# epruesse/SINA

Hardware: AMD Instinct MI355X
Metric: aligned sequences/sec (whole node), 100k full-length 16S vs SILVA-NR-scale ref (higher is better)
Workload: dtype f32

## Files before the change

### sina_amd/csrc/api.hip

```cpp
#include <algorithm>
#include <cmath>
#include <cstdlib>
#include <cstring>

#include "common.h"
#include "ctx.h"

namespace sina_hip {

static thread_local std::string g_last_error;
static thread_local bool g_last_error_is_limit = false;
void set_error(const std::string &msg) {
    g_last_error = msg;
    g_last_error_is_limit = false;
}
void set_limit_error(const std::string &msg) {
    g_last_error = msg;
    g_last_error_is_limit = true;
}

int make_streams(sina_hip_ctx *c) {
    SH_CHECK(hipStreamCreateWithFlags(&c->stream, hipStreamNonBlocking));
    SH_CHECK(hipStreamCreateWithFlags(&c->stream_dp, hipStreamNonBlocking));
    return 0;
// ... 123 lines not shown

    const uint64_t tb_budget_cells = tb_plane_budget(c) / tb_cell_bytes(forbid);
    const uint32_t slots = dp_wave_slots(c, pl.geom.B);
    const uint32_t range_q = (uint32_t)strtoul(test_knob("dp_range_q").c_str(), nullptr, 10);
    auto nodes_of = [&](uint32_t q) { return g->node_off[q + 1] - g->node_off[q]; };
    HostPrep hp;
    for (uint32_t q0 = qa, q1; q0 < qb; q0 = q1) {
        q1 = dbg ? q0 + 1 : dp_cut_range(nodes_of, q0, qb, Lp, tb_budget_cells, slots);
        if (range_q != 0) q1 = std::min(q1, q0 + range_q);
        if (prep_range(g, qoff, q0, q1, Lp, pl.W, &hp, pp.on ? pp.kappa64 : 0.f, spill_q)) return 1;
        const uint32_t bq = q1 - q0;
        const uint64_t nbase = g->node_off[q0], nn = g->node_off[q1] - nbase;
        const uint64_t ebase = g->edge_off[q0], ne = g->edge_off[q1] - ebase;
        const uint64_t qbase = qoff[q0], nqm = qoff[q1] - qbase;
        if (c->qd.reserve(sizeof(QDesc) * bq) || c->rec.reserve(sizeof(uint4) * nn) || c->node_pos.reserve(4 * nn) ||
            c->pred.reserve(4 * std::max<uint64_t>(ne, 1)) || c->succ_minpos.reserve(4 * nn) ||
            c->qmask.reserve(nqm) || (pp.on && c->rgain.reserve(8 * nn)))
            return 1;
        hipStream_t s = c->stream;
        SH_CHECK(hipMemcpyAsync(c->qd.p, hp.qd.data(), sizeof(QDesc) * bq, hipMemcpyHostToDevice, s));
        SH_CHECK(hipMemcpyAsync(c->rec.p, hp.rec.data(), sizeof(uint4) * nn, hipMemcpyHostToDevice, s));
        SH_CHECK(hipMemcpyAsync(c->node_pos.p, g->node_pos + nbase, 4 * nn, hipMemcpyHostToDevice, s));
        if (ne) SH_CHECK(hipMemcpyAsync(c->pred.p, hp.pred.data(), 4 * ne, hipMemcpyHostToDevice, s));
        if (g->succ_minpos)
            SH_CHECK(hipMemcpyAsync(c->succ_minpos.p, g->succ_minpos + nbase, 4 * nn, hipMemcpyHostToDevice, s));
        SH_CHECK(hipMemcpyAsync(c->qmask.p, qmask + qbase, nqm, hipMemcpyHostToDevice, s));
        PrunePlan pp_launch = pp;
        if (!hp.rgain_ok) pp_launch.on = 0;
        if (pp.on) SH_CHECK(hipMemcpyAsync(c->rgain.p, hp.rgain.data(), 8 * nn, hipMemcpyHostToDevice, s));
        if (profile_batch) {
            if (!g->self_score16) SH_FAIL("align_graphs: node_score16 without self_score16");
            if (weighted_scheme(p)) SH_FAIL("align_graphs: a profile batch takes no positional weights (scoring_scheme_profile)");
            if (c->prof16.reserve(64 * std::max<uint64_t>(nn, 1)) || c->self16.reserve(64)) return 1;
            SH_CHECK(hipMemcpyAsync(c->prof16.p, g->node_score16 + 16 * nbase, 64 * nn, hipMemcpyHostToDevice, s));
            SH_CHECK(hipMemcpyAsync(c->self16.p, g->self_score16, 64, hipMemcpyHostToDevice, s));
        }
        DpLaunch l;
        l.qd = hp.qd.data();
// ... 360 lines not shown
```

### sina_amd/csrc/common.h

```cpp
#pragma once

#include <hip/hip_runtime.h>
#include <stdint.h>

#include <algorithm>
#include <atomic>
#include <mutex>
#include <string>
#include <vector>

#include <cstdio>
#include <cstdlib>
#include <ctime>

#include "sina_hip.h"

namespace sina_hip {

void set_error(const std::string &msg);
void set_limit_error(const std::string &msg);

inline std::string test_knob(const char *key) {
    const char *e = getenv("SINA_HIP_TEST");
    if (!e) return std::string();
// ... 115 lines not shown

struct QDesc {
    uint64_t node_off;
    uint64_t edge_off;
    uint64_t q_off;
    uint64_t tb_off;
    uint64_t spill_off;
    uint32_t N, L;
    uint32_t n_spill;
    uint32_t erec_off;
    uint32_t first_sink;
    uint32_t gmin;
};
static_assert(sizeof(QDesc) == 64, "uploaded as an array");

constexpr uint32_t kRecSink = 1u << 16;
constexpr uint32_t kRecFence = 1u << 17;
constexpr int kRecDistShift = 18;
constexpr uint32_t kRecDistFar = 63u;
constexpr uint32_t kRowNone = 0xFFFFFFFFu;
constexpr uint32_t kRowSpilled = 0x80000000u;
constexpr uint32_t kPredSpilled = 0x80000000u;
constexpr uint32_t kMaxSpillRows = 32768;
constexpr int kFarLds = 192;
__host__ __device__ inline uint32_t dp_slot_segment(uint32_t n_rows) {
    const uint32_t s = (n_rows + 15u) / 16u;
    return s < 256u ? 256u : s;
}

struct EdgeRec {
// ... 72 lines not shown
    const uint2 *reach;
    int prune;
    float prune_rho;
    uint32_t prune_amax;
    float scout_bias;
    float *scout_u;
    const uint16_t *chain_rows;
    const uint32_t *chain_sizes;
    uint32_t chain_ncap;
};

struct BtArgs {
    const QDesc *qd;
    const uint4 *rec;
    const uint32_t *pred;
    const uint32_t *node_pos;
    const void *tb;
    const DpResult *res;
    const float *weights;
    uint32_t n_weights;
    const uint32_t *wset;
    sina_hip_align_out *out;
    uint32_t *out_pos;
    uint32_t nq, width, Lp;
    float ms;
    int overhang;
    int lazy_sidx;
    const uint8_t *qmask;
    int lowercase;
    uint32_t asm_cap;
// ... 55 lines not shown
```

### sina_amd/csrc/ctx.h

```cpp
#pragma once

#include <atomic>
#include <algorithm>
#include <condition_variable>
#include <cmath>
#include <cstring>

#include "dp_plan.h"
#include "identity_plan.h"

struct sina_hip_store {
    sina_hip::DevBuf ref_ab, ref_off, idx_off, idx_ids;
    std::vector<uint64_t> ref_off_host;
    std::atomic<bool> ref_off_host_ready{false};
    uint32_t n_refs = 0, width = 0, k = 0, nofast = 0;
    uint64_t n_postings = 0, total_bases = 0;
    bool have_refs = false, have_index = false;
    sina_hip::DevBuf dense_id, dense_bits;
    uint32_t n_dense = 0, dense_words = 0;
    std::atomic<bool> dense_ready{false};
    sina_hip::DevBuf name_rank, name_inv;
    bool have_name_order = false;
    sina_hip::DevBuf pair_ent;
    uint32_t n_pair_ent = 0;
// ... 90 lines not shown

struct sina_hip_ctx {
    int device = 0;
    int n_cu = 256;
    hipStream_t stream = nullptr;
    hipStream_t stream_dp = nullptr;
    std::mutex mu;
    hipEvent_t ev[14];

    sina_hip_store *st = nullptr;
    bool owns_store = false;

    sina_hip::DevBuf qd, order, rec, node_pos, pred, succ_minpos, qmask, spill, edge, res, weights, out, out_pos, dbg;
    sina_hip::DevBuf prof16, self16;
    sina_hip::DevBuf rgain;
    sina_hip::DevBuf wset;
    sina_hip::DevBuf wide_in, wide_planes;
    uint64_t path_queries[sina_hip::kNumSlowPaths] = {};
    sina_hip::KernelUse use[sina_hip::kNumKernelUse];
    sina_hip::DevBuf k_big_keys, k_big_tmp;
    sina_hip::DevBuf scout, scout_u;
    sina_hip::HostBuf h_res;
    void *last_tb = nullptr;
    bool last_scout = false;
    uint32_t last_bq = 0, last_prune_step = 0;
    uint32_t last_kernel = 0;
    sina_hip::DevBuf k_qoff, k_scores, k_out_ids, k_out_scores, k_out_n, k_tmp0, k_tmp1, k_tmp2;
    sina_hip::DevBuf g_fam_ids, g_fam_off, g_tmp0, g_tmp1, g_tmp2, g_tmp3, g_sizes, g_wtab;
    sina_hip::DevBuf s_qab, s_qoff, s_cand, s_coff, s_out;
    sina_hip::DevBuf m_out, m_n;
    sina_hip::DevBuf r_keys, r_ids, r_scores, r_n, r_flag, r_cnt;
    sina_hip::InplaceCount inplace[sina_hip::kNumInplace] = {{24, sina_hip::kUsePairsInplace, 12},
                                                             {sina_hip::identity_row_bytes(1), sina_hip::kUseIdentityInplace, 13}};
    sina_hip::HostBuf h_out, h_out_pos;
    sina_hip::HostBuf h_stage[12];
    float wtab_fs_weight = NAN;
    uint32_t prof_ncap = 0;

    size_t lds_budget = 0;

    static constexpr int kNumScratch = 50;
    static_assert(kNumScratch <= 64, "sina_hip_store::cap_hint is too short");
    void scratch(sina_hip::DevBuf **all) {
        sina_hip::DevBuf *list[kNumScratch] = {&qd, &rec, &node_pos, &pred, &succ_minpos, &qmask, &spill, &res,
                                               &weights, &out, &out_pos, &k_qoff, &k_scores, &k_out_ids,
                                               &k_out_scores, &k_out_n, &k_tmp0, &k_tmp1, &k_tmp2, &g_fam_ids,
                                               &g_fam_off, &g_tmp0, &g_tmp1, &g_tmp2, &g_tmp3, &g_sizes, &g_wtab, &order,
                                               &s_qab, &s_qoff, &s_cand, &s_coff, &s_out, &edge, &prof16, &self16, &rgain,
                                               &scout, &scout_u, &wset, &m_out, &m_n, &r_keys, &r_ids, &r_scores, &r_n, &r_flag,
                                               &r_cnt, &inplace[sina_hip::kInplacePairs].rows, &inplace[sina_hip::kInplaceIdentity].rows};
        for (int i = 0; i < kNumScratch; i++) all[i] = list[i];
    }
    void publish_hints() {
        sina_hip::DevBuf *all[kNumScratch];
        scratch(all);
        for (int i = 0; i < kNumScratch; i++) {
            size_t seen = st->cap_hint[i].load(std::memory_order_relaxed);
            while (all[i]->cap > seen && !st->cap_hint[i].compare_exchange_weak(seen, all[i]->cap, std::memory_order_relaxed)) {
            }
        }
    }
    void bind_hints() {
        sina_hip::DevBuf *all[kNumScratch];
        scratch(all);
        for (int i = 0; i < kNumScratch; i++) all[i]->hint = &st->cap_hint[i];
        for (int i = 0; i < sina_hip::kNumInplace; i++) inplace[i].hint = &st->inplace_rows_hint[i];
    }
    int prewarm(int kind) {
        sina_hip::DevBuf *search[] = {&k_qoff, &k_scores, &k_out_ids, &k_out_scores, &k_out_n, &k_tmp0, &k_tmp1, &k_tmp2, &qmask,
                                      &s_qab, &r_keys, &r_ids, &r_scores, &r_n, &r_flag, &r_cnt};
        sina_hip::DevBuf *align[] = {&qd, &order, &rec, &node_pos, &pred, &succ_minpos, &qmask, &spill, &edge, &res, &weights, &out,
                                     &out_pos, &g_fam_ids, &g_fam_off, &g_tmp0, &g_tmp1, &g_tmp2, &g_tmp3, &g_sizes, &g_wtab, &rgain, &scout, &scout_u,
                                     &prof16, &self16, &wset, &inplace[sina_hip::kInplacePairs].rows, &inplace[sina_hip::kInplaceIdentity].rows};
        sina_hip::DevBuf *compare[] = {&s_qab, &s_qoff, &s_cand, &s_coff, &s_out, &m_out, &m_n, &r_keys, &r_ids, &r_scores, &r_n, &r_flag, &r_cnt};
        sina_hip::DevBuf **list = kind == 0 ? search : (kind == 1 ? align : compare);
        const size_t n = kind == 0 ? sizeof search / sizeof *search : (kind == 1 ? sizeof align / sizeof *align : sizeof compare / sizeof *compare);
        for (size_t i = 0; i < n; i++) {
            const size_t want = list[i]->hint ? list[i]->hint->load(std::memory_order_relaxed) : 0;
            if (want > list[i]->cap && list[i]->reserve_exact(want)) return 1;
        }
        for (auto &ic : inplace)
            if (kind == 1 && ic.h_rows.reserve(ic.hint->load(std::memory_order_relaxed))) return 1;
        return 0;
    }
    void free_all() {
        if (st && st->wedged.load(std::memory_order_relaxed)) return;
// ... 379 lines not shown
```

### sina_amd/csrc/dp_launch.hip

```cpp
#include <algorithm>
#include <cmath>
#include <cstdlib>
#include <cstring>

#include "common.h"
#include "ctx.h"

namespace sina_hip {

bool pick_geom(uint32_t maxL, DpGeom *g) {
    int t = 0, b = 0;
    if (const std::string ov = test_knob("geom"); ov.empty() || sscanf(ov.c_str(), "%d,%d", &t, &b) != 2) t = b = 0;
    return dp_geom_for(maxL, t, b, g);
}

int plan_dp(sina_hip_ctx *c, uint32_t maxL, DpPlan *pl) {
    DpGeom g;
    if (!pick_geom(maxL, &g)) SH_FAIL_LIMIT("align: query longer than SINA_HIP_MAX_QUERY_LEN bases");
    dp_ring_plan(g, c->lds_budget, pl);
    if (pl->W < 1) SH_FAIL("align: LDS cannot hold one DP row");
    return 0;
}

PrunePlan prune_plan(const sina_hip_align_params *p, float wmax, float wmin, uint32_t maxL, bool profile_batch) {
// ... 78 lines not shown
    }
    a->ms = -p->match_score;
    a->mms = -p->mismatch_score;
    a->gp = p->gap_penalty;
    a->gpe = p->gap_ext_penalty;
    a->prof16 = l.profile_batch ? c->prof16.as<float>() : nullptr;
    c->last_bq = l.bq;
    c->last_prune_step = pp.on ? pp.amax : 0u;
    a->reach = pp.on ? c->rgain.as<uint2>() : nullptr;
    a->prune = pp.on;
    a->prune_amax = pp.amax;
    a->below_init = (!weighted && !forbid && dp_below_init(sums.max_n, a->gp, a->gpe)) ? 1 : 0;
    b->qd = a->qd;
    b->rec = a->rec;
    b->pred = a->pred;
    b->node_pos = a->node_pos;
    b->res = a->res;
    b->weights = a->weights;
    b->n_weights = a->n_weights;
    b->wset = a->wset;
    b->out = c->out.as<sina_hip_align_out>();
    b->out_pos = c->out_pos.as<uint32_t>();
    b->nq = l.bq;
    b->width = l.width;
    b->Lp = (uint32_t)pl.geom.Lp();
    b->ms = a->ms;
    b->overhang = p->overhang;
    b->lazy_sidx = forbid ? 0 : 1;
    b->qmask = a->qmask;
    b->lowercase = p->lowercase;
// ... 267 lines not shown
```

### sina_amd/csrc/dp_plan.h

```cpp
#pragma once

#include <cassert>
#include <cmath>
#include <cstring>
#include <string_view>
#include <unordered_map>

#include "common.h"

namespace sina_hip {

enum DpKernelKind : uint32_t {
    kDpKernelNone = SINA_DP_KERNEL_NONE,
    kDpKernelSimple = SINA_DP_KERNEL_SIMPLE,
    kDpKernelSimpleSkip = SINA_DP_KERNEL_SIMPLE_SKIP,
    kDpKernelGenericBelow = SINA_DP_KERNEL_GENERIC_BELOW,
    kDpKernelGeneric = SINA_DP_KERNEL_GENERIC,
    kDpKernelWeighted = SINA_DP_KERNEL_WEIGHTED,
    kDpKernelForbid = SINA_DP_KERNEL_FORBID,
    kDpKernelWeightedForbid = SINA_DP_KERNEL_WEIGHTED_FORBID,
};
inline DpKernelKind dp_kernel_kind(bool weighted, bool forbid, bool below_init, float gp, float gpe, bool generic_only,
                                   bool profile_batch, bool prune_on, uint32_t n_strips) {
    if (!weighted && !forbid && below_init && gp >= gpe && !generic_only && !profile_batch)
// ... 203 lines not shown
    std::nth_element(ratios.begin(), ratios.begin() + (std::ptrdiff_t)at, ratios.end());
    const float rho_guard_seen = ratios[at] - 0.015f;
    if (!(rho_seen > 0.f)) return;
    *rho = rho_seen < *rho ? rho_seen : 0.5f * (*rho + rho_seen);
    *rho = std::min(0.99f, std::max(0.05f, *rho));
    *rho_guard = rho_guard_seen < *rho_guard ? rho_guard_seen : 0.5f * (*rho_guard + rho_guard_seen);
    *rho_guard = std::min(0.99f, std::max(0.05f, *rho_guard));
}

struct HostPrep {
    std::vector<QDesc> qd;
    std::vector<uint4> rec;
    std::vector<uint2> rgain;
    bool rgain_ok = true;
    std::vector<uint32_t> pred;
    std::vector<uint32_t> last;
};

inline int prep_range(const sina_hip_graph_batch *g, const uint64_t *qoff, uint32_t q0, uint32_t q1, int Lp, int W,
                       HostPrep *hp, float kappa64, uint32_t *spill_q) {
    const uint64_t nbase = g->node_off[q0], ebase = g->edge_off[q0];
    const uint64_t nn = g->node_off[q1] - nbase;
    hp->qd.resize(q1 - q0);
    hp->rec.resize(nn);
    hp->rgain.assign(kappa64 > 0.f ? nn : 0, uint2{0u, 0u});
    hp->rgain_ok = true;
    hp->pred.resize(g->edge_off[q1] - ebase + 8);
    uint64_t tb_cells = 0, spill_rows = 0;
    uint32_t erec_cursor = 0;
    for (uint32_t q = q0; q < q1; q++) {
        QDesc &d = hp->qd[q - q0];
        const uint64_t no = g->node_off[q], eo = g->edge_off[q];
        const uint32_t N = (uint32_t)(g->node_off[q + 1] - no);
        d.node_off = no - nbase;
        d.erec_off = erec_cursor;
        erec_cursor += dp_edge_entries(N);
        d.edge_off = eo - ebase;
        d.q_off = qoff[q] - qoff[q0];
        d.tb_off = tb_cells;
// ... 46 lines not shown
                for (int x = 0; x < W; x++)
                    if (free_at[x] <= m) {
                        slot = x;
                        break;
                    }
            if (slot >= 0) {
                free_at[slot] = last[m];
                rec[m].w = (uint32_t)slot;
            } else {
                rec[m].w = kRowSpilled | nsp++;
            }
        }
        for (uint32_t m = 0; m < N; m++) {
            uint32_t first_far = 0;
            uint32_t dist = po[m + 1] > po[m] ? 0u : kRecDistFar;
            for (uint32_t e = po[m]; e < po[m + 1]; e++) {
                const uint32_t p = g->pred[eo + e];
                const uint32_t pw = rec[p].w == kRowNone ? 0u : rec[p].w;
                const bool sp = (pw & kRowSpilled) != 0;
                if (sp && first_far == 0) first_far = e - po[m] + 1;
                dist = std::max(dist, m - p);
                hp->pred[d.edge_off + e] = p | ((pw & 0x7FFFu) << 16) | (sp ? kPredSpilled : 0u);
            }
            rec[m].z |= (first_far << 24) | (std::min(dist, kRecDistFar) << kRecDistShift);
        }
        if (nsp > kMaxSpillRows) {
            if (spill_q) *spill_q = q;
            SH_FAIL_LIMIT("align_graphs: too many spill rows for one query");
        }
        if (kappa64 > 0.f) {
            uint2 *rg = hp->rgain.data() + d.node_off;
            const uint32_t *pos = g->node_pos + no;
            bool ok = true;
            for (uint32_t m = 0; m < N && ok; m++) {
                if (m > 0 && pos[m] < pos[m - 1]) ok = false;
                for (uint32_t e = po[m]; e < po[m + 1] && ok; e++)
                    if (pos[g->pred[eo + e]] >= pos[m]) ok = false;
            }
            if (!ok) hp->rgain_ok = false;
// ... 44 lines not shown
```

### sina_amd/csrc/graph_build.hip

```cpp
#include <algorithm>
#include <cstring>
#include <type_traits>

#include "common.h"
#include "ctx.h"

namespace sina_hip {
namespace {

#ifndef SINA_GRAPH_THREADS
#define SINA_GRAPH_THREADS 512
#endif
#ifndef SINA_GRAPH_MINWAVES
#define SINA_GRAPH_MINWAVES 8
#endif
constexpr int kGT = SINA_GRAPH_THREADS;
constexpr uint32_t kNoPrev = 0xFFFFu;
constexpr int kMaxFam = kFamilyMax;
#ifndef SINA_GRAPH_KTC
#define SINA_GRAPH_KTC 128
#endif
#ifndef SINA_GRAPH_TNW
#define SINA_GRAPH_TNW 512
#endif
// ... 13 lines not shown
#define GP_FLUSH
#endif

struct GraphArgs {
    const uint32_t *ref_ab;
    const uint64_t *ref_off;
    const uint32_t *fam_ids;
    const uint64_t *fam_off;
    const uint64_t *pred_off;
    const float *wtab;
    uint4 *rec;
    uint32_t *node_pos;
    uint32_t *succ_min;
    uint32_t *far_mark;
    uint32_t *pred;
    uint32_t *sizes;
    uint16_t *chain_rows;
    uint32_t width, ncap;
    uint32_t tile_bytes;
    uint32_t bitmap_off;
    uint32_t member_off;
    uint32_t member_cap;
    uint32_t fam_cap;
    int W;
    int want_smin;
    uint2 *reach;
    float kappa64;
};

struct Member {
// ... 546 lines not shown
            }
            rec[i].w = w;
            if (in_lds) codeL[i] = w;
        }
        if (tid == 0) {
            sz[kBuiltN] = N;
            sz[kBuiltEdges] = E;
            sz[kBuiltSpill] = tot;
            sz[kBuiltStatus] = (tot > kMaxSpillRows) ? kBuiltSpillCap : 0u;
            sz[kBuiltFirstSink] = s_tmp[kGT / 64 + 1];
            sz[kBuiltChainLen] = mb[0].len;
        }
    }
    __syncthreads();
    GP(10)
    for (uint32_t i = tid; i < N; i += kGT) {
        const uint4 r = rec[i];
        const uint32_t np = r.z & 0xFFu;
        uint32_t first_far = 0;
        uint32_t dist = np ? 0u : kRecDistFar;
        for (uint32_t x = 0; x < np; x++) {
            const uint32_t pa = pred[r.x + x];
            uint32_t pw = in_lds ? codeL[pa] : rec[pa].w;
            if (pw == kRowNone) pw = 0;
            const bool sp = (pw & kRowSpilled) != 0;
            if (sp && first_far == 0) first_far = x + 1;
            dist = max(dist, i - pa);
            pred[r.x + x] = pa | ((pw & 0x7FFFu) << 16) | (sp ? kPredSpilled : 0u);
        }
        rec[i].z = r.z | (first_far << 24) | (min(dist, kRecDistFar) << kRecDistShift);
    }
    GP(11)
    if (a.reach != nullptr) {
        uint2 *rg = a.reach + (size_t)q * a.ncap;
        uint32_t *cw = in_lds ? codeL : (a.want_smin ? last : smin);
        if (tid == 0) s_tmp[kGT / 64 + 2] = 0xFFFFFFFFu;
        __syncthreads();
        for (uint32_t i = tid; i < N; i += kGT) {
            const uint32_t pos = node_pos[i];
            if (i > 0 && node_pos[i - 1] == pos) continue;
            uint32_t mx = 0;
            for (uint32_t j = i; j < N && node_pos[j] == pos; j++) {
                mx = max(mx, prune_gain_units(__uint_as_float(rec[j].y), a.kappa64));
                cw[j] = 0;
            }
// ... 63 lines not shown
    }
    uint32_t ncap = std::min<uint32_t>(65535, 12288);
    for (int attempt = 0;; attempt++) {
        uint64_t pred_total = 0;
        for (uint32_t q = 0; q < bq; q++) {
            bg->pred_off[q] = pred_total;
            pred_total += elems[q] + 8;
        }
        const size_t glds_tables = graph_lds_bytes(c->st->width, max_f);
        const size_t glds = graph_lds_total(c->st->width, max_f);
        if (glds > 160 * 1024) SH_FAIL_LIMIT("align_families: family too wide for the device DAG build");
        if (c->g_fam_ids.reserve(4 * std::max<uint64_t>(foff[bq], 1)) || c->g_fam_off.reserve(8 * ((uint64_t)bq + 1)) ||
            c->g_tmp1.reserve(8 * (uint64_t)bq) ||
            c->rec.reserve(sizeof(uint4) * (uint64_t)bq * ncap) || c->node_pos.reserve(4 * (uint64_t)bq * ncap) ||
            c->succ_minpos.reserve(4 * (uint64_t)bq * ncap) || c->g_tmp3.reserve(4 * (uint64_t)bq * ncap) ||
            c->pred.reserve(4 * pred_total) || c->g_sizes.reserve(4 * kBuiltWords * (uint64_t)bq) ||
            c->scout.reserve(2 * (uint64_t)bq * ncap) ||
            (kappa64 > 0.f && c->rgain.reserve(8 * (uint64_t)bq * ncap)))
            return 1;
        if (upload(c, 1, c->g_fam_ids.p, fam_ids + fam_off[q0], 4 * foff[bq], s) ||
            upload(c, 2, c->g_fam_off.p, foff.data(), 8 * ((uint64_t)bq + 1), s) ||
            upload(c, 3, c->g_tmp1.p, bg->pred_off.data(), 8 * (uint64_t)bq, s))
            return 1;
        GraphArgs ga;
        ga.ref_ab = c->st->ref_ab.as<uint32_t>();
        ga.ref_off = c->st->ref_off.as<uint64_t>();
        ga.fam_ids = c->g_fam_ids.as<uint32_t>();
        ga.fam_off = c->g_fam_off.as<uint64_t>();
        ga.pred_off = c->g_tmp1.as<uint64_t>();
        ga.wtab = c->g_wtab.as<float>();
        ga.rec = c->rec.as<uint4>();
        ga.node_pos = c->node_pos.as<uint32_t>();
        ga.succ_min = c->succ_minpos.as<uint32_t>();
        ga.far_mark = c->g_tmp3.as<uint32_t>();
        ga.pred = c->pred.as<uint32_t>();
        ga.sizes = c->g_sizes.as<uint32_t>();
        ga.chain_rows = c->scout.as<uint16_t>();
        ga.width = c->st->width;
        ga.ncap = ncap;
        ga.bitmap_off = (uint32_t)graph_bitmap_off(max_f);
        ga.tile_bytes = ga.bitmap_off;
        ga.member_off = (uint32_t)glds_tables;
        ga.member_cap = (uint32_t)graph_member_cap(max_f);
        ga.fam_cap = max_f;
        ga.W = W;
        ga.want_smin = want_smin ? 1 : 0;
        ga.reach = kappa64 > 0.f ? c->rgain.as<uint2>() : nullptr;
        ga.kappa64 = kappa64;
        if (allow_full_lds(reinterpret_cast<const void *>(family_graph_kernel))) return 1;
        bg->sizes.resize(kBuiltWords * (size_t)bq);
// ... 1 lines not shown
            heavy_launch hl(c, s, kHeavyGraph);
            SH_CHECK(hipEventRecord(c->ev[6], hl.stream()));
            hipLaunchKernelGGL(family_graph_kernel, dim3(bq), dim3(kGT), glds, hl.stream(), ga);
            SH_CHECK(hipGetLastError());
            SH_CHECK(hipEventRecord(c->ev[7], hl.stream()));
            if (hl.done()) return 1;
        }
        if (download(c, 4, c->g_sizes.p, 4 * kBuiltWords * (uint64_t)bq, s)) return 1;
        SH_CHECK(wait_stream(c, s));
        memcpy(bg->sizes.data(), c->h_stage[4].p, 4 * kBuiltWords * (uint64_t)bq);
        float gms = 0;
        SH_CHECK(hipEventElapsedTime(&gms, c->ev[6], c->ev[7]));
        {
            uint64_t bytes = 0;
            for (uint32_t q = 0; q < bq; q++)
                bytes += 4 * elems[q] + (uint64_t)bg->sizes[kBuiltWords * q + kBuiltN] * (16 + 4 + (kappa64 > 0.f ? 8 : 0)) +
                         4 * (uint64_t)bg->sizes[kBuiltWords * q + kBuiltEdges];
            std::lock_guard<std::mutex> slk(c->st->stats_mu);
            c->st->stats.graph_ms += gms;
            c->st->stats.graph_bytes += bytes;
            c->st->stats.graph_launches++;
        }
        uint32_t need_n = 0;
        for (uint32_t q = 0; q < bq; q++) {
            const uint32_t status = bg->sizes[kBuiltWords * q + kBuiltStatus];
            if (status == kBuiltNodeCap) need_n = std::max(need_n, bg->sizes[kBuiltWords * q + kBuiltN]);
            if (status == kBuiltSpillCap) SH_FAIL_LIMIT("align_families: too many spill rows for one query");
        }
        if (!need_n) break;
        if (attempt >= 3 || need_n > 65535u) SH_FAIL_LIMIT("align_families: family DAG exceeds device limits");
        ncap = std::min<uint32_t>(65535, need_n + need_n / 8 + 16);
// ... 113 lines not shown
```

### sina_amd/csrc/profile_build.hip

```cpp
#include <algorithm>
#include <cstring>
#include <limits>

#include "common.h"
#include "ctx.h"

namespace sina_hip {
namespace {

constexpr int kPT = 512;
constexpr uint32_t kTileMax = 6144;
constexpr uint32_t kLdsSlack = 256;

struct Shares {
    float v[6];
};
__host__ __device__ inline Shares shares_of_mask(uint32_t mask) {
    Shares b;
    for (int i = 0; i < 6; i++) b.v[i] = 0.f;
    const int order = ((mask >> 0) & 1) + ((mask >> 1) & 1) + ((mask >> 2) & 1) + ((mask >> 3) & 1);
    if (order > 0) {
        const float val = 1.f / (float)order;
        for (int i = 0; i < 4; i++)
            if (mask & (1u << i)) b.v[i] = val;
// ... 7 lines not shown
            if (i == j) res += match * a.v[i] * b.v[j];
            else res += mismatch * a.v[i] * b.v[j];
        }
    return res + gap * a.v[4] + gap_ext * a.v[5];
}

struct ProfileArgs {
    const uint32_t *ref_ab;
    const uint64_t *ref_off;
    const uint32_t *fam_ids;
    const uint64_t *fam_off;
    uint4 *rec;
    uint32_t *node_pos;
    uint32_t *succ_min;
    uint32_t *pred;
    float *prof16;
    uint32_t *sizes;
    uint32_t width, ncap, pred_stride;
    uint32_t tile_nodes;
    uint32_t bitmap_off;
    uint32_t member_off;
    float match, mismatch, gap, gap_ext;
};

struct PMember {
    uint64_t beg;
    uint32_t len;
    uint32_t cur, curn;
    uint32_t pad_;
};
// ... 76 lines not shown
            sz[kBuiltEdges] = sz[kBuiltSpill] = 0;
            sz[kBuiltStatus] = kBuiltNodeCap;
            sz[kBuiltFirstSink] = sz[kBuiltGmin] = 0;
        }
        return;
    }
    auto rank = [&](uint32_t pos) -> uint32_t {
        return (uint32_t)wrank[pos >> 5] + __popc(bitmap[pos >> 5] & ((1u << (pos & 31)) - 1u));
    };

    {
        uint4 *rec = a.rec + (size_t)q * a.ncap;
        uint32_t *node_pos = a.node_pos + (size_t)q * a.ncap;
        uint32_t *smin = a.succ_min + (size_t)q * a.ncap;
        uint32_t *pred = a.pred + (size_t)q * a.pred_stride;
        for (uint32_t w = tid; w < nwords; w += kPT) {
            uint32_t bits = bitmap[w], n = wrank[w];
            while (bits) {
                const uint32_t pos = w * 32u + (uint32_t)(__ffs(bits) - 1);
                bits &= bits - 1u;
                node_pos[n] = pos;
                if (n > 0) smin[n - 1] = pos;
                n++;
            }
        }
        for (uint32_t n = tid; n < N; n += kPT) {
            uint4 r;
            r.x = n > 0 ? n - 1u : 0u;
            r.y = 0u;
            r.z = (n > 0 ? 1u : 0u) | (n + 1 == N ? kRecSink : 0u) | ((n > 0 ? 1u : kRecDistFar) << kRecDistShift);
            r.w = kRowNone;
            rec[n] = r;
            if (n + 1 < N) pred[n] = n;
        }
        if (tid == 0) {
            smin[N - 1] = 1000000u;
            sz[kBuiltN] = N;
            sz[kBuiltEdges] = N - 1u;
            sz[kBuiltSpill] = 0;
            sz[kBuiltStatus] = 0;
            sz[kBuiltFirstSink] = N - 1u;
            sz[kBuiltGmin] = 0;
        }
    }

    float *prof = a.prof16 + 16 * ((size_t)q * a.ncap);
    for (uint32_t n0 = 0; n0 < N; n0 += T) {
// ... 166 lines not shown
        c->g_sizes.reserve(4 * kBuiltWords * (uint64_t)n))
        return 1;
    if (upload(c, 1, c->g_fam_ids.p, fam_ids + fam_off[q0], 4 * foff[n], s) ||
        upload(c, 2, c->g_fam_off.p, foff.data(), 8 * ((uint64_t)n + 1), s))
        return 1;
    if (allow_full_lds(reinterpret_cast<const void *>(family_profile_kernel))) return 1;
    uint32_t ncap = c->prof_ncap ? c->prof_ncap : 4096u;
    uint32_t max_n = 1;
    const uint32_t forced_tile = (uint32_t)strtoul(test_knob("profile_tile").c_str(), nullptr, 10);
    for (int attempt = 0;; attempt++) {
        ProfileLds lds;
        if (!profile_lds(c->st->width, max_f, ncap, forced_tile, &lds)) SH_FAIL_LIMIT("align_profiles: family too wide for the device profile build");
        const uint32_t pred_stride = ncap + 8;
        if (c->rec.reserve(sizeof(uint4) * (uint64_t)n * ncap) || c->node_pos.reserve(4 * (uint64_t)n * ncap) ||
            c->succ_minpos.reserve(4 * (uint64_t)n * ncap) || c->pred.reserve(4 * (uint64_t)n * pred_stride) ||
            c->prof16.reserve(64 * (uint64_t)n * ncap))
            return 1;
        ProfileArgs pa;
        pa.ref_ab = c->st->ref_ab.as<uint32_t>();
        pa.ref_off = c->st->ref_off.as<uint64_t>();
        pa.fam_ids = c->g_fam_ids.as<uint32_t>();
        pa.fam_off = c->g_fam_off.as<uint64_t>();
        pa.rec = c->rec.as<uint4>();
        pa.node_pos = c->node_pos.as<uint32_t>();
        pa.succ_min = c->succ_minpos.as<uint32_t>();
        pa.pred = c->pred.as<uint32_t>();
        pa.prof16 = c->prof16.as<float>();
        pa.sizes = c->g_sizes.as<uint32_t>();
        pa.width = c->st->width;
        pa.ncap = ncap;
        pa.pred_stride = pred_stride;
        pa.tile_nodes = lds.tile_nodes;
        pa.bitmap_off = lds.bitmap_off;
        pa.member_off = lds.member_off;
        pa.match = -p->match_score;
        pa.mismatch = -p->mismatch_score;
        pa.gap = p->gap_penalty;
        pa.gap_ext = p->gap_ext_penalty;
        {
            heavy_launch hl(c, s, kHeavyGraph);
            SH_CHECK(hipEventRecord(c->ev[6], hl.stream()));
// ... 9 lines not shown
        float gms = 0;
        SH_CHECK(hipEventElapsedTime(&gms, c->ev[6], c->ev[7]));
        uint32_t need_n = 0;
        uint64_t nodes = 0;
        max_n = 1;
        for (uint32_t q = 0; q < n; q++) {
            const uint32_t N = bg->sizes[kBuiltWords * q + kBuiltN];
            if (bg->sizes[kBuiltWords * q + kBuiltStatus] == kBuiltNodeCap) need_n = std::max(need_n, N);
            else nodes += N;
            max_n = std::max(max_n, N);
        }
        {
            std::lock_guard<std::mutex> slk(c->st->stats_mu);
            c->st->stats.graph_ms += gms;
            if (!need_n) {
                c->st->stats.graph_bytes += 4 * bases + nodes * (16 + 4 + 4 + 4 + 64);
                c->st->stats.graph_launches++;
            }
        }
        if (!need_n) break;
        if (attempt >= 3 || need_n > 65535u) SH_FAIL_LIMIT("align_profiles: family profile exceeds device limits (more than 65535 nodes)");
        ncap = std::min<uint32_t>(65535, need_n + need_n / 8 + 16);
    }
    c->prof_ncap = std::max(c->prof_ncap, std::min<uint32_t>(65535, max_n + max_n / 8 + 16));
    bg->ncap = ncap;
    bg->pred_off.resize(n);
    for (uint32_t q = 0; q < n; q++) bg->pred_off[q] = (uint64_t)q * (ncap + 8);
    return 0;
}

}
// ... 67 lines not shown
```

### sina_amd/csrc/traceback.hip

```cpp
#include <cstdlib>
#include <type_traits>

#include "common.h"
#include "dp_plan.h"

namespace sina_hip {

namespace {

template <bool LAZY>
struct BtDirect {
    using cell_t = typename std::conditional<LAZY, uint16_t, uint32_t>::type;
    static constexpr bool writes = true;
    const cell_t *tb;
    const uint4 *recs;
    const uint32_t *node_pos, *preds;
    uint32_t Lp;
    __device__ BtDirect(const BtArgs &a, const QDesc &d)
        : tb(reinterpret_cast<const cell_t *>(a.tb) + d.tb_off), recs(a.rec + d.node_off), node_pos(a.node_pos + d.node_off),
          preds(a.pred + d.edge_off), Lp(a.Lp) {}
    __device__ uint32_t cell(uint32_t row, uint32_t col) const { return (uint32_t)tb[(size_t)row * Lp + col]; }
    __device__ uint4 rec(uint32_t row) const {
        uint4 rx = recs[row];
        rx.w = node_pos[row];
        return rx;
    }
    __device__ uint32_t pred(uint32_t, uint32_t pb, uint32_t e) const { return preds[pb + e] & 0xffffu; }
};

constexpr int kBtRows = 64, kBtCols = 32;
template <bool LAZY>
struct BtWindow {
    using cell_t = typename BtDirect<LAZY>::cell_t;
    static constexpr uint32_t kAlign = 16 / sizeof(cell_t);
    struct Lds {
        cell_t cell[kBtRows][kBtCols];
        uint4 rec[kBtRows];
        uint4 pred[kBtRows];
    };
    BtDirect<LAZY> g;
    Lds &w;
    uint32_t N, lane;
    bool writes;
    uint32_t wr0 = 0x80000000u, wc0 = 0;
    __device__ BtWindow(const BtArgs &a, const QDesc &d, Lds &lds, uint32_t lane_)
        : g(a, d), w(lds), N(d.N), lane(lane_), writes(lane_ == 0) {}
    __device__ void refill(uint32_t row, uint32_t col) {
        __syncthreads();
        wr0 = row + 1 >= (uint32_t)kBtRows ? row + 1 - kBtRows : 0u;
        const uint32_t ctop = (col & ~(kAlign - 1)) + kAlign;
        wc0 = ctop >= (uint32_t)kBtCols ? ctop - kBtCols : 0u;
        const uint32_t x = wr0 + lane;
        if (x < N) {
            const uint4 *src = reinterpret_cast<const uint4 *>(g.tb + (size_t)x * g.Lp + wc0);
            uint4 *dst = reinterpret_cast<uint4 *>(&w.cell[lane][0]);
#pragma unroll
            for (uint32_t i = 0; i < kBtCols / kAlign; i++) dst[i] = src[i];
            const uint4 rx = g.rec(x);
            w.rec[lane] = rx;
            const uint32_t np = rx.z & 0xffu;
            uint4 pe = {0u, 0u, 0u, 0u};
            if (np > 0) pe.x = g.preds[rx.x];
            if (np > 1) pe.y = g.preds[rx.x + 1];
            if (np > 2) pe.z = g.preds[rx.x + 2];
            if (np > 3) pe.w = g.preds[rx.x + 3];
            w.pred[lane] = pe;
        }
        __syncthreads();
    }
    __device__ bool in_rows(uint32_t row) const { return row - wr0 < (uint32_t)kBtRows; }
    __device__ uint32_t cell(uint32_t row, uint32_t col) {
        if (!(in_rows(row) && col - wc0 < (uint32_t)kBtCols)) refill(row, col);
        return (uint32_t)w.cell[row - wr0][col - wc0];
    }
    __device__ uint4 rec(uint32_t row) const {
        if (in_rows(row)) return w.rec[row - wr0];
        return g.rec(row);
    }
    __device__ uint32_t pred(uint32_t row, uint32_t pb, uint32_t e) const {
        if (e < 4 && in_rows(row)) {
            const uint4 pe = w.pred[row - wr0];
            return (e == 0 ? pe.x : (e == 1 ? pe.y : (e == 2 ? pe.z : pe.w))) & 0xffffu;
        }
        return g.pred(row, pb, e);
    }
};

template <bool LAZY, class Mem>
__device__ __forceinline__ void walk_query(const BtArgs &a, uint32_t q, const QDesc &d, Mem &mem) {
    const DpResult r = a.res[q];
    sina_hip_align_out o;
    o.status = r.status;
    o.end_m = r.end_m;
    o.end_s = r.end_s;
    o.raw = r.raw;
    o.sum_weight = 0.f;
    o.aligned_bases = 0;
    o.cutoff_head = o.cutoff_tail = 0;
    o.n_out = 0;
    o.assembled = o.nast_total = o.nast_longest = o.nast_last_run = 0;
// ... 1 lines not shown
        if (mem.writes) a.out[q] = o;
        return;
    }
    uint32_t *out = a.out_pos + d.q_off;
    const uint32_t width = a.width;
    uint32_t m = r.end_m, s = r.end_s;
    uint32_t n = 0;
    const uint32_t send = d.L - 1;
    auto emit = [&](uint32_t p) {
        if (mem.writes) out[n] = p;
        n++;
    };

    const int tail = (int)(send - s);
    o.cutoff_tail = tail;
    uint32_t c = mem.cell(m, s);
    uint4 rm = mem.rec(m);
    if (tail && a.overhang != SINA_OVERHANG_REMOVE) {
        int pos = (a.overhang == SINA_OVERHANG_ATTACH) ? (int)(width - 1 - rm.w - (uint32_t)tail) : 0;
        for (int i = 0; i < tail; i++) {
            const int p = pos++;
            emit((uint32_t)(p > 0 ? p : 0));
        }
    }
    const uint8_t *qmb = a.qmask + d.q_off;
    const float *wts = a.weights;
    if (wts != nullptr && a.wset != nullptr) wts += (size_t)a.wset[q] * a.n_weights;
    auto mscore_at = [&](const uint4 &rx, uint32_t si) -> float {
        if (a.self16 != nullptr) return a.self16[qmb[si] & 0xfu];
        const float wgt = __uint_as_float(rx.y);
        if (wts != nullptr) {
            const uint32_t nw1 = a.n_weights - 1;
            return a.ms * wts[rx.w < nw1 ? rx.w : nw1] * wgt;
        }
        return a.ms * wgt;
    };
    unsigned int pos = width - 1 - rm.w;
    float sum_weight = 0.f;
    int aligned = 0;
    emit(pos);
    aligned++;
    sum_weight = sum_weight + mscore_at(rm, s);

    constexpr uint32_t ext_bit = LAZY ? kTb16Ext : kTbExt;
    auto gapm_idx = [&](uint32_t x, uint32_t col) -> uint32_t {
        for (uint32_t guard = 0; guard < 65536u; ++guard) {
            const uint32_t cx = mem.cell(x, col);
            const uint4 rx = mem.rec(x);
            const uint32_t np = rx.z & 0xffu;
            if (np == 0) return 0u;
            const uint32_t lastp = mem.pred(x, rx.x, np - 1);
            if (LAZY ? !(cx & kTb16XLast) : (cx & kTbOpLast) != 0) return lastp;
            x = lastp;
        }
        return 0u;
    };
    auto midx_raw = [&](uint32_t cc, uint32_t row, uint32_t pb) -> uint32_t {
        if (!LAZY) return cc >> 16;
        const uint32_t t = cc & kTbTypeMask;
        if (t == kTbIns) return row;
        if (t == kTbNone) return 0u;
        return mem.pred(row, pb, cc >> kTb16OrdShift);
    };
    auto sidx_of = [&](uint32_t cc, uint32_t row, uint32_t col) -> uint32_t {
        if (!LAZY) return cc & kTbSMask;
        const uint32_t t = cc & kTbTypeMask;
        if (t == kTbNone) return 0u;
        if (t == kTbMatch) return col - 1;
        if (t == kTbDel) return col;
        uint32_t k = col - 1;
        while (k > 0 && (mem.cell(row, k) & kTbTypeMask) == kTbIns) --k;
        return k;
    };
    auto is_deletion_at = [&](uint32_t cc, uint32_t col) -> bool {
        return LAZY ? (cc & kTbTypeMask) == kTbDel : (cc & kTbSMask) == col;
    };
    uint32_t npred_m = rm.z & 0xffu;
    while (s != 0 && npred_m != 0) {
        const uint32_t snew = sidx_of(c, m, s);
        const uint32_t vm = midx_raw(c, m, rm.x);
        m = (c & ext_bit) ? gapm_idx(vm, s) : vm;
        c = mem.cell(m, snew);
        if (snew != 0 && is_deletion_at(c, snew)) {
            const uint32_t vm2 = midx_raw(c, m, mem.rec(m).x);
            m = (c & ext_bit) ? gapm_idx(vm2, snew) : vm2;
            c = mem.cell(m, snew);
        }
        rm = mem.rec(m);
        npred_m = rm.z & 0xffu;
        pos = width - 1 - rm.w;
        while (s != snew) {
            --s;
            emit(pos);
            aligned++;
            sum_weight = sum_weight + mscore_at(rm, s);
        }
    }
    if (s != 0) {
        o.cutoff_head = (int)s;
        if (a.overhang == SINA_OVERHANG_ATTACH) {
            while (s-- != 0) {
                ++pos;
                emit((width - 1 < pos) ? width - 1 : pos);
// ... 160 lines not shown
```

Before: 294,600.

## Pack first four predecessors per node and fetch row state together in traceback

Adds a per-node pred4 array holding the first four predecessor indices as packed 16-bit values. It is built in the graph, profile and host prep paths and uploaded alongside the other graph buffers. Traceback now loads the cell, record and packed predecessors in one step, so the serial chain of dependent pred[] gathers becomes independent loads, and the LDS window shrinks from uint4 to uint2 per row. In exchange it costs extra memory, an extra host-to-device copy per range, and more work when building graphs.

```diff
diff --git a/sina_amd/csrc/api.hip b/sina_amd/csrc/api.hip
--- a/sina_amd/csrc/api.hip
+++ b/sina_amd/csrc/api.hip
@@ -161,7 +161,7 @@
         const uint64_t ebase = g->edge_off[q0], ne = g->edge_off[q1] - ebase;
         const uint64_t qbase = qoff[q0], nqm = qoff[q1] - qbase;
         if (c->qd.reserve(sizeof(QDesc) * bq) || c->rec.reserve(sizeof(uint4) * nn) || c->node_pos.reserve(4 * nn) ||
-            c->pred.reserve(4 * std::max<uint64_t>(ne, 1)) || c->succ_minpos.reserve(4 * nn) ||
+            c->pred.reserve(4 * std::max<uint64_t>(ne, 1)) || c->pred4.reserve(sizeof(uint2) * nn) || c->succ_minpos.reserve(4 * nn) ||
             c->qmask.reserve(nqm) || (pp.on && c->rgain.reserve(8 * nn)))
             return 1;
         hipStream_t s = c->stream;
@@ -169,6 +169,7 @@
         SH_CHECK(hipMemcpyAsync(c->rec.p, hp.rec.data(), sizeof(uint4) * nn, hipMemcpyHostToDevice, s));
         SH_CHECK(hipMemcpyAsync(c->node_pos.p, g->node_pos + nbase, 4 * nn, hipMemcpyHostToDevice, s));
         if (ne) SH_CHECK(hipMemcpyAsync(c->pred.p, hp.pred.data(), 4 * ne, hipMemcpyHostToDevice, s));
+        SH_CHECK(hipMemcpyAsync(c->pred4.p, hp.pred4.data(), sizeof(uint2) * nn, hipMemcpyHostToDevice, s));
         if (g->succ_minpos)
             SH_CHECK(hipMemcpyAsync(c->succ_minpos.p, g->succ_minpos + nbase, 4 * nn, hipMemcpyHostToDevice, s));
         SH_CHECK(hipMemcpyAsync(c->qmask.p, qmask + qbase, nqm, hipMemcpyHostToDevice, s));
diff --git a/sina_amd/csrc/common.h b/sina_amd/csrc/common.h
--- a/sina_amd/csrc/common.h
+++ b/sina_amd/csrc/common.h
@@ -153,6 +153,9 @@
 };
 static_assert(sizeof(QDesc) == 64, "uploaded as an array");
 
+__host__ __device__ inline uint2 pred4_pack(uint32_t p0, uint32_t p1, uint32_t p2, uint32_t p3) {
+    return uint2{(p0 & 0xffffu) | (p1 << 16), (p2 & 0xffffu) | (p3 << 16)};
+}
 constexpr uint32_t kRecSink = 1u << 16;
 constexpr uint32_t kRecFence = 1u << 17;
 constexpr int kRecDistShift = 18;
@@ -255,6 +258,7 @@
     const QDesc *qd;
     const uint4 *rec;
     const uint32_t *pred;
+    const uint2 *pred4;
     const uint32_t *node_pos;
     const void *tb;
     const DpResult *res;
diff --git a/sina_amd/csrc/ctx.h b/sina_amd/csrc/ctx.h
--- a/sina_amd/csrc/ctx.h
+++ b/sina_amd/csrc/ctx.h
@@ -128,6 +128,7 @@
     sina_hip::DevBuf qd, order, rec, node_pos, pred, succ_minpos, qmask, spill, edge, res, weights, out, out_pos, dbg;
     sina_hip::DevBuf prof16, self16;
     sina_hip::DevBuf rgain;
+    sina_hip::DevBuf pred4;
     sina_hip::DevBuf wset;
     sina_hip::DevBuf wide_in, wide_planes;
     uint64_t path_queries[sina_hip::kNumSlowPaths] = {};
@@ -153,7 +154,7 @@
 
     size_t lds_budget = 0;
 
-    static constexpr int kNumScratch = 50;
+    static constexpr int kNumScratch = 51;
     static_assert(kNumScratch <= 64, "sina_hip_store::cap_hint is too short");
     void scratch(sina_hip::DevBuf **all) {
         sina_hip::DevBuf *list[kNumScratch] = {&qd, &rec, &node_pos, &pred, &succ_minpos, &qmask, &spill, &res,
@@ -162,7 +163,7 @@
                                                &g_fam_off, &g_tmp0, &g_tmp1, &g_tmp2, &g_tmp3, &g_sizes, &g_wtab, &order,
                                                &s_qab, &s_qoff, &s_cand, &s_coff, &s_out, &edge, &prof16, &self16, &rgain,
                                                &scout, &scout_u, &wset, &m_out, &m_n, &r_keys, &r_ids, &r_scores, &r_n, &r_flag,
-                                               &r_cnt, &inplace[sina_hip::kInplacePairs].rows, &inplace[sina_hip::kInplaceIdentity].rows};
+                                               &r_cnt, &inplace[sina_hip::kInplacePairs].rows, &inplace[sina_hip::kInplaceIdentity].rows, &pred4};
         for (int i = 0; i < kNumScratch; i++) all[i] = list[i];
     }
     void publish_hints() {
@@ -183,7 +184,7 @@
     int prewarm(int kind) {
         sina_hip::DevBuf *search[] = {&k_qoff, &k_scores, &k_out_ids, &k_out_scores, &k_out_n, &k_tmp0, &k_tmp1, &k_tmp2, &qmask,
                                       &s_qab, &r_keys, &r_ids, &r_scores, &r_n, &r_flag, &r_cnt};
-        sina_hip::DevBuf *align[] = {&qd, &order, &rec, &node_pos, &pred, &succ_minpos, &qmask, &spill, &edge, &res, &weights, &out,
+        sina_hip::DevBuf *align[] = {&qd, &order, &rec, &node_pos, &pred, &pred4, &succ_minpos, &qmask, &spill, &edge, &res, &weights, &out,
                                      &out_pos, &g_fam_ids, &g_fam_off, &g_tmp0, &g_tmp1, &g_tmp2, &g_tmp3, &g_sizes, &g_wtab, &rgain, &scout, &scout_u,
                                      &prof16, &self16, &wset, &inplace[sina_hip::kInplacePairs].rows, &inplace[sina_hip::kInplaceIdentity].rows};
         sina_hip::DevBuf *compare[] = {&s_qab, &s_qoff, &s_cand, &s_coff, &s_out, &m_out, &m_n, &r_keys, &r_ids, &r_scores, &r_n, &r_flag, &r_cnt};
diff --git a/sina_amd/csrc/dp_launch.hip b/sina_amd/csrc/dp_launch.hip
--- a/sina_amd/csrc/dp_launch.hip
+++ b/sina_amd/csrc/dp_launch.hip
@@ -116,6 +116,7 @@
     b->qd = a->qd;
     b->rec = a->rec;
     b->pred = a->pred;
+    b->pred4 = c->pred4.as<uint2>();
     b->node_pos = a->node_pos;
     b->res = a->res;
     b->weights = a->weights;
diff --git a/sina_amd/csrc/dp_plan.h b/sina_amd/csrc/dp_plan.h
--- a/sina_amd/csrc/dp_plan.h
+++ b/sina_amd/csrc/dp_plan.h
@@ -241,6 +241,7 @@
     std::vector<uint2> rgain;
     bool rgain_ok = true;
     std::vector<uint32_t> pred;
+    std::vector<uint2> pred4;
     std::vector<uint32_t> last;
 };
 
@@ -250,6 +251,7 @@
     const uint64_t nn = g->node_off[q1] - nbase;
     hp->qd.resize(q1 - q0);
     hp->rec.resize(nn);
+    hp->pred4.resize(nn);
     hp->rgain.assign(kappa64 > 0.f ? nn : 0, uint2{0u, 0u});
     hp->rgain_ok = true;
     hp->pred.resize(g->edge_off[q1] - ebase + 8);
@@ -326,8 +328,10 @@
         for (uint32_t m = 0; m < N; m++) {
             uint32_t first_far = 0;
             uint32_t dist = po[m + 1] > po[m] ? 0u : kRecDistFar;
+            uint32_t p4[4] = {0u, 0u, 0u, 0u};
             for (uint32_t e = po[m]; e < po[m + 1]; e++) {
                 const uint32_t p = g->pred[eo + e];
+                if (e - po[m] < 4u) p4[e - po[m]] = p;
                 const uint32_t pw = rec[p].w == kRowNone ? 0u : rec[p].w;
                 const bool sp = (pw & kRowSpilled) != 0;
                 if (sp && first_far == 0) first_far = e - po[m] + 1;
@@ -335,6 +339,7 @@
                 hp->pred[d.edge_off + e] = p | ((pw & 0x7FFFu) << 16) | (sp ? kPredSpilled : 0u);
             }
             rec[m].z |= (first_far << 24) | (std::min(dist, kRecDistFar) << kRecDistShift);
+            hp->pred4[d.node_off + m] = pred4_pack(p4[0], p4[1], p4[2], p4[3]);
         }
         if (nsp > kMaxSpillRows) {
             if (spill_q) *spill_q = q;
diff --git a/sina_amd/csrc/graph_build.hip b/sina_amd/csrc/graph_build.hip
--- a/sina_amd/csrc/graph_build.hip
+++ b/sina_amd/csrc/graph_build.hip
@@ -51,6 +51,7 @@
     uint32_t *succ_min;
     uint32_t *far_mark;
     uint32_t *pred;
+    uint2 *pred4;
     uint32_t *sizes;
     uint16_t *chain_rows;
     uint32_t width, ncap;
@@ -627,11 +628,13 @@
     }
     __syncthreads();
     GP(10)
+    uint2 *pred4 = a.pred4 + (size_t)q * a.ncap;
     for (uint32_t i = tid; i < N; i += kGT) {
         const uint4 r = rec[i];
         const uint32_t np = r.z & 0xFFu;
         uint32_t first_far = 0;
         uint32_t dist = np ? 0u : kRecDistFar;
+        uint32_t p4[4] = {0u, 0u, 0u, 0u};
         for (uint32_t x = 0; x < np; x++) {
             const uint32_t pa = pred[r.x + x];
             uint32_t pw = in_lds ? codeL[pa] : rec[pa].w;
@@ -640,8 +643,13 @@
             if (sp && first_far == 0) first_far = x + 1;
             dist = max(dist, i - pa);
             pred[r.x + x] = pa | ((pw & 0x7FFFu) << 16) | (sp ? kPredSpilled : 0u);
+            if (x == 0) p4[0] = pa;
+            else if (x == 1) p4[1] = pa;
+            else if (x == 2) p4[2] = pa;
+            else if (x == 3) p4[3] = pa;
         }
         rec[i].z = r.z | (first_far << 24) | (min(dist, kRecDistFar) << kRecDistShift);
+        pred4[i] = pred4_pack(p4[0], p4[1], p4[2], p4[3]);
     }
     GP(11)
     if (a.reach != nullptr) {
@@ -735,7 +743,7 @@
             c->g_tmp1.reserve(8 * (uint64_t)bq) ||
             c->rec.reserve(sizeof(uint4) * (uint64_t)bq * ncap) || c->node_pos.reserve(4 * (uint64_t)bq * ncap) ||
             c->succ_minpos.reserve(4 * (uint64_t)bq * ncap) || c->g_tmp3.reserve(4 * (uint64_t)bq * ncap) ||
-            c->pred.reserve(4 * pred_total) || c->g_sizes.reserve(4 * kBuiltWords * (uint64_t)bq) ||
+            c->pred.reserve(4 * pred_total) || c->pred4.reserve(sizeof(uint2) * (uint64_t)bq * ncap) || c->g_sizes.reserve(4 * kBuiltWords * (uint64_t)bq) ||
             c->scout.reserve(2 * (uint64_t)bq * ncap) ||
             (kappa64 > 0.f && c->rgain.reserve(8 * (uint64_t)bq * ncap)))
             return 1;
@@ -755,6 +763,7 @@
         ga.succ_min = c->succ_minpos.as<uint32_t>();
         ga.far_mark = c->g_tmp3.as<uint32_t>();
         ga.pred = c->pred.as<uint32_t>();
+        ga.pred4 = c->pred4.as<uint2>();
         ga.sizes = c->g_sizes.as<uint32_t>();
         ga.chain_rows = c->scout.as<uint16_t>();
         ga.width = c->st->width;
@@ -786,7 +795,7 @@
         {
             uint64_t bytes = 0;
             for (uint32_t q = 0; q < bq; q++)
-                bytes += 4 * elems[q] + (uint64_t)bg->sizes[kBuiltWords * q + kBuiltN] * (16 + 4 + (kappa64 > 0.f ? 8 : 0)) +
+                bytes += 4 * elems[q] + (uint64_t)bg->sizes[kBuiltWords * q + kBuiltN] * (16 + 4 + 8 + (kappa64 > 0.f ? 8 : 0)) +
                          4 * (uint64_t)bg->sizes[kBuiltWords * q + kBuiltEdges];
             std::lock_guard<std::mutex> slk(c->st->stats_mu);
             c->st->stats.graph_ms += gms;
diff --git a/sina_amd/csrc/profile_build.hip b/sina_amd/csrc/profile_build.hip
--- a/sina_amd/csrc/profile_build.hip
+++ b/sina_amd/csrc/profile_build.hip
@@ -45,6 +45,7 @@
     uint32_t *node_pos;
     uint32_t *succ_min;
     uint32_t *pred;
+    uint2 *pred4;
     float *prof16;
     uint32_t *sizes;
     uint32_t width, ncap, pred_stride;
@@ -151,6 +152,7 @@
         uint32_t *node_pos = a.node_pos + (size_t)q * a.ncap;
         uint32_t *smin = a.succ_min + (size_t)q * a.ncap;
         uint32_t *pred = a.pred + (size_t)q * a.pred_stride;
+        uint2 *pred4 = a.pred4 + (size_t)q * a.ncap;
         for (uint32_t w = tid; w < nwords; w += kPT) {
             uint32_t bits = bitmap[w], n = wrank[w];
             while (bits) {
@@ -168,6 +170,7 @@
             r.z = (n > 0 ? 1u : 0u) | (n + 1 == N ? kRecSink : 0u) | ((n > 0 ? 1u : kRecDistFar) << kRecDistShift);
             r.w = kRowNone;
             rec[n] = r;
+            pred4[n] = pred4_pack(n > 0 ? n - 1u : 0u, 0u, 0u, 0u);
             if (n + 1 < N) pred[n] = n;
         }
         if (tid == 0) {
@@ -364,6 +367,7 @@
         const uint32_t pred_stride = ncap + 8;
         if (c->rec.reserve(sizeof(uint4) * (uint64_t)n * ncap) || c->node_pos.reserve(4 * (uint64_t)n * ncap) ||
             c->succ_minpos.reserve(4 * (uint64_t)n * ncap) || c->pred.reserve(4 * (uint64_t)n * pred_stride) ||
+            c->pred4.reserve(sizeof(uint2) * (uint64_t)n * ncap) ||
             c->prof16.reserve(64 * (uint64_t)n * ncap))
             return 1;
         ProfileArgs pa;
@@ -375,6 +379,7 @@
         pa.node_pos = c->node_pos.as<uint32_t>();
         pa.succ_min = c->succ_minpos.as<uint32_t>();
         pa.pred = c->pred.as<uint32_t>();
+        pa.pred4 = c->pred4.as<uint2>();
         pa.prof16 = c->prof16.as<float>();
         pa.sizes = c->g_sizes.as<uint32_t>();
         pa.width = c->st->width;
@@ -414,7 +419,7 @@
             std::lock_guard<std::mutex> slk(c->st->stats_mu);
             c->st->stats.graph_ms += gms;
             if (!need_n) {
-                c->st->stats.graph_bytes += 4 * bases + nodes * (16 + 4 + 4 + 4 + 64);
+                c->st->stats.graph_bytes += 4 * bases + nodes * (16 + 4 + 4 + 4 + 8 + 64);
                 c->st->stats.graph_launches++;
             }
         }
diff --git a/sina_amd/csrc/traceback.hip b/sina_amd/csrc/traceback.hip
--- a/sina_amd/csrc/traceback.hip
+++ b/sina_amd/csrc/traceback.hip
@@ -7,6 +7,17 @@
 namespace sina_hip {
 
 namespace {
+
+struct BtAt {
+    uint32_t c;
+    uint4 r;
+    uint2 p4;
+    __device__ uint32_t npred() const { return r.z & 0xffu; }
+    __device__ uint32_t pred_near(uint32_t e) const {
+        const uint32_t w = (e & 2u) ? p4.y : p4.x;
+        return (e & 1u) ? w >> 16 : w & 0xffffu;
+    }
+};
 
 template <bool LAZY>
 struct BtDirect {
@@ -14,18 +25,28 @@
     static constexpr bool writes = true;
     const cell_t *tb;
     const uint4 *recs;
+    const uint2 *pred4;
     const uint32_t *node_pos, *preds;
     uint32_t Lp;
     __device__ BtDirect(const BtArgs &a, const QDesc &d)
-        : tb(reinterpret_cast<const cell_t *>(a.tb) + d.tb_off), recs(a.rec + d.node_off), node_pos(a.node_pos + d.node_off),
-          preds(a.pred + d.edge_off), Lp(a.Lp) {}
+        : tb(reinterpret_cast<const cell_t *>(a.tb) + d.tb_off), recs(a.rec + d.node_off), pred4(a.pred4 + d.node_off),
+          node_pos(a.node_pos + d.node_off), preds(a.pred + d.edge_off), Lp(a.Lp) {}
     __device__ uint32_t cell(uint32_t row, uint32_t col) const { return (uint32_t)tb[(size_t)row * Lp + col]; }
     __device__ uint4 rec(uint32_t row) const {
         uint4 rx = recs[row];
         rx.w = node_pos[row];
         return rx;
     }
-    __device__ uint32_t pred(uint32_t, uint32_t pb, uint32_t e) const { return preds[pb + e] & 0xffffu; }
+    __device__ BtAt at(uint32_t row, uint32_t col) const {
+        BtAt x;
+        x.c = cell(row, col);
+        x.r = recs[row];
+        x.r.w = node_pos[row];
+        x.p4 = pred4[row];
+        asm volatile("" : "+v"(x.c), "+v"(x.r.x), "+v"(x.r.y), "+v"(x.r.z), "+v"(x.r.w), "+v"(x.p4.x), "+v"(x.p4.y));
+        return x;
+    }
+    __device__ uint32_t pred_far(uint32_t pb, uint32_t e) const { return preds[pb + e] & 0xffffu; }
 };
 
 constexpr int kBtRows = 64, kBtCols = 32;
@@ -36,7 +57,7 @@
     struct Lds {
         cell_t cell[kBtRows][kBtCols];
         uint4 rec[kBtRows];
-        uint4 pred[kBtRows];
+        uint2 pred[kBtRows];
     };
     BtDirect<LAZY> g;
     Lds &w;
@@ -56,15 +77,8 @@
             uint4 *dst = reinterpret_cast<uint4 *>(&w.cell[lane][0]);
 #pragma unroll
             for (uint32_t i = 0; i < kBtCols / kAlign; i++) dst[i] = src[i];
-            const uint4 rx = g.rec(x);
-            w.rec[lane] = rx;
-            const uint32_t np = rx.z & 0xffu;
-            uint4 pe = {0u, 0u, 0u, 0u};
-            if (np > 0) pe.x = g.preds[rx.x];
-            if (np > 1) pe.y = g.preds[rx.x + 1];
-            if (np > 2) pe.z = g.preds[rx.x + 2];
-            if (np > 3) pe.w = g.preds[rx.x + 3];
-            w.pred[lane] = pe;
+            w.rec[lane] = g.rec(x);
+            w.pred[lane] = g.pred4[x];
         }
         __syncthreads();
     }
@@ -73,17 +87,14 @@
         if (!(in_rows(row) && col - wc0 < (uint32_t)kBtCols)) refill(row, col);
         return (uint32_t)w.cell[row - wr0][col - wc0];
     }
-    __device__ uint4 rec(uint32_t row) const {
-        if (in_rows(row)) return w.rec[row - wr0];
-        return g.rec(row);
-    }
-    __device__ uint32_t pred(uint32_t row, uint32_t pb, uint32_t e) const {
-        if (e < 4 && in_rows(row)) {
-            const uint4 pe = w.pred[row - wr0];
-            return (e == 0 ? pe.x : (e == 1 ? pe.y : (e == 2 ? pe.z : pe.w))) & 0xffffu;
-        }
-        return g.pred(row, pb, e);
-    }
+    __device__ BtAt at(uint32_t row, uint32_t col) {
+        BtAt x;
+        x.c = cell(row, col);
+        x.r = w.rec[row - wr0];
+        x.p4 = w.pred[row - wr0];
+        return x;
+    }
+    __device__ uint32_t pred_far(uint32_t pb, uint32_t e) const { return g.pred_far(pb, e); }
 };
 
 template <bool LAZY, class Mem>
@@ -115,8 +126,8 @@
 
     const int tail = (int)(send - s);
     o.cutoff_tail = tail;
-    uint32_t c = mem.cell(m, s);
-    uint4 rm = mem.rec(m);
+    BtAt cur = mem.at(m, s);
+    uint4 rm = cur.r;
     if (tail && a.overhang != SINA_OVERHANG_REMOVE) {
         int pos = (a.overhang == SINA_OVERHANG_ATTACH) ? (int)(width - 1 - rm.w - (uint32_t)tail) : 0;
         for (int i = 0; i < tail; i++) {
@@ -144,24 +155,24 @@
     sum_weight = sum_weight + mscore_at(rm, s);
 
     constexpr uint32_t ext_bit = LAZY ? kTb16Ext : kTbExt;
+    auto pred_of = [&](const BtAt &x, uint32_t e) -> uint32_t { return e < 4u ? x.pred_near(e) : mem.pred_far(x.r.x, e); };
     auto gapm_idx = [&](uint32_t x, uint32_t col) -> uint32_t {
         for (uint32_t guard = 0; guard < 65536u; ++guard) {
-            const uint32_t cx = mem.cell(x, col);
-            const uint4 rx = mem.rec(x);
-            const uint32_t np = rx.z & 0xffu;
+            const BtAt ax = mem.at(x, col);
+            const uint32_t np = ax.npred();
             if (np == 0) return 0u;
-            const uint32_t lastp = mem.pred(x, rx.x, np - 1);
-            if (LAZY ? !(cx & kTb16XLast) : (cx & kTbOpLast) != 0) return lastp;
+            const uint32_t lastp = pred_of(ax, np - 1);
+            if (LAZY ? !(ax.c & kTb16XLast) : (ax.c & kTbOpLast) != 0) return lastp;
             x = lastp;
         }
         return 0u;
     };
-    auto midx_raw = [&](uint32_t cc, uint32_t row, uint32_t pb) -> uint32_t {
-        if (!LAZY) return cc >> 16;
-        const uint32_t t = cc & kTbTypeMask;
+    auto midx_raw = [&](const BtAt &x, uint32_t row) -> uint32_t {
+        if (!LAZY) return x.c >> 16;
+        const uint32_t t = x.c & kTbTypeMask;
         if (t == kTbIns) return row;
         if (t == kTbNone) return 0u;
-        return mem.pred(row, pb, cc >> kTb16OrdShift);
+        return pred_of(x, x.c >> kTb16OrdShift);
     };
     auto sidx_of = [&](uint32_t cc, uint32_t row, uint32_t col) -> uint32_t {
         if (!LAZY) return cc & kTbSMask;
@@ -178,16 +189,16 @@
     };
     uint32_t npred_m = rm.z & 0xffu;
     while (s != 0 && npred_m != 0) {
-        const uint32_t snew = sidx_of(c, m, s);
-        const uint32_t vm = midx_raw(c, m, rm.x);
-        m = (c & ext_bit) ? gapm_idx(vm, s) : vm;
-        c = mem.cell(m, snew);
-        if (snew != 0 && is_deletion_at(c, snew)) {
-            const uint32_t vm2 = midx_raw(c, m, mem.rec(m).x);
-            m = (c & ext_bit) ? gapm_idx(vm2, snew) : vm2;
-            c = mem.cell(m, snew);
-        }
-        rm = mem.rec(m);
+        const uint32_t snew = sidx_of(cur.c, m, s);
+        const uint32_t vm = midx_raw(cur, m);
+        m = (cur.c & ext_bit) ? gapm_idx(vm, s) : vm;
+        cur = mem.at(m, snew);
+        if (snew != 0 && is_deletion_at(cur.c, snew)) {
+            const uint32_t vm2 = midx_raw(cur, m);
+            m = (cur.c & ext_bit) ? gapm_idx(vm2, snew) : vm2;
+            cur = mem.at(m, snew);
+        }
+        rm = cur.r;
         npred_m = rm.z & 0xffu;
         pos = width - 1 - rm.w;
         while (s != snew) {
```

New measurement: 300,900 (median of 6 runs). 1.02x the previous value.
